# grossmanlev/FL-distributed-delay

Measured on AMD Instinct MI355X. Metric: simulated worker-steps/sec (node) @1024 workers, delay 50; aggregation HBM GB/s, higher is better.
Workload: dtype f32

## Files before the change

### fl-distributed-delay_amd/csrc/gemm_core.h

```cpp
#pragma once
#include <type_traits>

#include "common.h"

namespace flsim {

constexpr int GK = 16;

__device__ __forceinline__ int kc_swz(int row) { return (4 - ((row >> 2) & 3)) & 3; }

template <int ROWS>
struct KCTile {
    static constexpr int FLOATS = ROWS * GK;
    __device__ static inline int chunk_off(int row, int chunk) {
        return row * GK + 4 * (chunk ^ kc_swz(row));
    }
};
template <int ROWS>
struct KMTile {
    static constexpr int STRIDE = ROWS + 4;
    static constexpr int DUMMY = GK * STRIDE;
    static constexpr int FLOATS = GK * STRIDE + 4;
};

__device__ __forceinline__ f32x4 mfma16(float a, float b, f32x4 c) {
    return __builtin_amdgcn_mfma_f32_16x16x4f32(a, b, c, 0, 0, 0);
}

template <bool KC, int ROWS>
__device__ __forceinline__ f32x4 read_frag(const float* lds, int r0, int lane) {
    if constexpr (KC) {
        const int row = r0 + (lane & 15);
        return *reinterpret_cast<const f32x4*>(lds + KCTile<ROWS>::chunk_off(row, lane >> 4));
    } else {
        constexpr int S = KMTile<ROWS>::STRIDE;
        const int col = r0 + (lane & 15);
        const int k0 = 4 * (lane >> 4);
        f32x4 v;
        v.x = lds[(k0 + 0) * S + col];
        v.y = lds[(k0 + 1) * S + col];
        v.z = lds[(k0 + 2) * S + col];
        v.w = lds[(k0 + 3) * S + col];
        return v;
    }
}

template <bool KC, int ROWS>
__device__ __forceinline__ void store_unit(float* lds, int a, int b, f32x4 v) {
    if constexpr (KC) {
        *reinterpret_cast<f32x4*>(lds + KCTile<ROWS>::chunk_off(a, b)) = v;
    } else {
        *reinterpret_cast<f32x4*>(lds + a * KMTile<ROWS>::STRIDE + 4 * b) = v;
    }
}

template <int ROWS>
__device__ __forceinline__ void store_km_or_spare(float* lds, bool valid, int a, int b, f32x4 v) {
    const int off = valid ? a * KMTile<ROWS>::STRIDE + 4 * b : KMTile<ROWS>::DUMMY;
    *reinterpret_cast<f32x4*>(lds + off) = v;
}

template <bool KC, int ROWS>
constexpr int tile_floats() {
    if constexpr (KC) return KCTile<ROWS>::FLOATS;
    else return KMTile<ROWS>::FLOATS;
}


template <class E, class = void>
struct IsStaged : std::false_type {};
template <class E>
struct IsStaged<E, std::void_t<decltype(E::STAGED)>> : std::bool_constant<E::STAGED> {};

template <class E, class = void>
struct IsPartial : std::false_type {};
template <class E>
struct IsPartial<E, std::void_t<decltype(E::PARTIAL)>> : std::bool_constant<E::PARTIAL> {};

template <class EPI>
__device__ __forceinline__ void staged_store(const EPI& epi, const float* tile, int ld, int m0,
                                             int bm, int n0, int bn, int tid, int nt) {
    if constexpr (IsPartial<EPI>::value)
        epi.store_rows(tile, ld, m0, bm, n0, bn, tid, nt);
    else
        epi.store_rows(tile, ld, m0, bm, tid, nt);
}

template <class E, class = void>
struct HasPre : std::false_type {};
template <class E>
struct HasPre<E, std::void_t<decltype(E::PRE)>> : std::bool_constant<E::PRE> {};

#ifndef FLSIM_SINGLE_BUF
#define FLSIM_SINGLE_BUF 2
#endif

template <int FM, int FN, int WAVES_M, int WAVES_N, class AL, class BL, class EPI>
__global__ void __launch_bounds__(64 * WAVES_M * WAVES_N)
gemm_kernel(AL al, BL bl, EPI epi, int ksteps_total, int ksteps_per_split, int tiles_m,
            int tiles_n) {
    constexpr int BM = 16 * FM * WAVES_M;
    constexpr int BN = 16 * FN * WAVES_N;
    static_assert(AL::ROWS == BM, "A loader rows != BM");
    static_assert(BL::ROWS == BN, "B loader rows != BN");
    constexpr int A_FL = tile_floats<AL::KC, BM>();
    constexpr int B_FL = tile_floats<BL::KC, BN>();
    constexpr bool STAGED = IsStaged<EPI>::value;
    constexpr int STAGE_LD = BN + 4;
    constexpr bool SB = WAVES_M * WAVES_N <= FLSIM_SINGLE_BUF && !STAGED;
    constexpr int BASE_FL = (SB ? 1 : 2) * (A_FL + B_FL);
    constexpr int STAGE_BUDGET = BASE_FL > 8192 ? BASE_FL : 8192;
    constexpr int WROWS = 16 * FM;
    constexpr int WM_FIT = STAGE_BUDGET / (WROWS * STAGE_LD);
    constexpr int WM_PASS = WM_FIT < 1 ? 1 : (WM_FIT > WAVES_M ? WAVES_M : WM_FIT);
    constexpr int LDS_FL = STAGED && WM_PASS * WROWS * STAGE_LD > BASE_FL
                               ? WM_PASS * WROWS * STAGE_LD : BASE_FL;
    __shared__ __attribute__((aligned(16))) float lds[LDS_FL];

    const int tid = threadIdx.x;
    const int lane = tid & 63;
    const int wave = tid >> 6;
    const int wm = wave / WAVES_N;
    const int wn = wave % WAVES_N;
    const int gx = tiles_m, gy = tiles_n;
    const int nb = gridDim.x;
    const int b = blockIdx.x;
    const int q = nb / 8, r = nb % 8, xcd = b % 8;
    const int L = (xcd < r ? xcd * (q + 1) : r * (q + 1) + (xcd - r) * q) + b / 8;
    const int tn = L % gy;
    const int tm = (L / gy) % gx;
    const int tz = L / (gx * gy);
    const int m0 = tm * BM;
    const int n0 = tn * BN;
    const int ks0 = tz * ksteps_per_split;
    int ks1 = ks0 + ksteps_per_split;
    if (ks1 > ksteps_total) ks1 = ksteps_total;

    al.setup(m0, tid);
    bl.setup(n0, tid);

    f32x4 acc[FM][FN];
#pragma unroll
    for (int i = 0; i < FM; ++i)
#pragma unroll
        for (int j = 0; j < FN; ++j) acc[i][j] = f32x4{0.f, 0.f, 0.f, 0.f};

    float asum = 0.f;
    f32x4 ra[AL::UNITS];
    f32x4 rb[BL::UNITS];
    constexpr int BUF = A_FL + B_FL;

    if (ks0 < ks1) {
        al.load(ks0, ra);
        bl.load(ks0, rb);
        if constexpr (!SB) {
            al.store(lds, ra);
            bl.store(lds + A_FL, rb);
            if (ks0 + 1 < ks1) {
                al.load(ks0 + 1, ra);
                bl.load(ks0 + 1, rb);
            }
        }
    }
    __syncthreads();
    if constexpr (WAVES_M * WAVES_N == 8) {
        if (wave >= 4) __builtin_amdgcn_s_setprio(1);
    }
    int cur = 0;
    for (int ks = ks0; ks < ks1; ++ks) {
        if constexpr (SB) {
            al.store(lds, ra);
            bl.store(lds + A_FL, rb);
            if (ks + 1 < ks1) {
                al.load(ks + 1, ra);
                bl.load(ks + 1, rb);
            }
            __syncthreads();
        } else if (ks + 1 < ks1) {
            al.store(lds + (cur ^ 1) * BUF, ra);
            bl.store(lds + (cur ^ 1) * BUF + A_FL, rb);
            if (ks + 2 < ks1) {
                al.load(ks + 2, ra);
                bl.load(ks + 2, rb);
            }
        }
        const float* A = lds + (SB ? 0 : cur * BUF);
        const float* B = A + A_FL;
        if constexpr (EPI::ASUM) {
            static_assert(!AL::KC, "ASUM needs a k-major A tile");
            if (tn == 0 && tid < BM) {
#pragma unroll
                for (int k = 0; k < GK; ++k) asum += A[k * KMTile<BM>::STRIDE + tid];
            }
        }
        f32x4 af[FM], bf[FN];
#pragma unroll
        for (int i = 0; i < FM; ++i) af[i] = read_frag<AL::KC, BM>(A, wm * 16 * FM + 16 * i, lane);
#pragma unroll
        for (int j = 0; j < FN; ++j) bf[j] = read_frag<BL::KC, BN>(B, wn * 16 * FN + 16 * j, lane);
#pragma unroll
        for (int kk = 0; kk < 4; ++kk)
#pragma unroll
            for (int i = 0; i < FM; ++i)
#pragma unroll
                for (int j = 0; j < FN; ++j) acc[i][j] = mfma16(af[i][kk], bf[j][kk], acc[i][j]);
        __syncthreads();
        cur ^= 1;
    }

    if constexpr (EPI::ASUM) {
        if (tn == 0 && tid < BM) epi.asum(m0 + tid, tz, asum);
    }
    if constexpr (STAGED) {
        static_assert(BN == EPI::NCOL || (IsPartial<EPI>::value && EPI::NCOL % BN == 0),
                      "staged epilogue needs the full row in one block");
        constexpr int PASSES = (WAVES_M + WM_PASS - 1) / WM_PASS;
#pragma unroll 1
        for (int pass = 0; pass < PASSES; ++pass) {
            __syncthreads();
            if (wm / WM_PASS == pass) {
#pragma unroll
                for (int i = 0; i < FM; ++i)
#pragma unroll
                    for (int j = 0; j < FN; ++j) {
                        const int ml = (wm - pass * WM_PASS) * WROWS + 16 * i + 4 * (lane >> 4);
                        const int nl = wn * 16 * FN + 16 * j + (lane & 15);
#pragma unroll
                        for (int r = 0; r < 4; ++r)
                            lds[(ml + r) * STAGE_LD + nl] = epi.value(nl, acc[i][j][r]);
                    }
            }
            __syncthreads();
            const int wm_hi = (pass + 1) * WM_PASS < WAVES_M ? (pass + 1) * WM_PASS : WAVES_M;
            staged_store(epi, lds, STAGE_LD, m0 + pass * WM_PASS * WROWS,
                         (wm_hi - pass * WM_PASS) * WROWS, n0, BN, tid, 64 * WAVES_M * WAVES_N);
        }
    } else if constexpr (HasPre<EPI>::value) {
#pragma unroll
        for (int i = 0; i < FM; ++i) {
            const int m = m0 + wm * 16 * FM + 16 * i + 4 * (lane >> 4);
            const int nb = n0 + wn * 16 * FN + (lane & 15);
            f32x4 pre[FN];
#pragma unroll
            for (int j = 0; j < FN; ++j) pre[j] = epi.pre4(m, nb + 16 * j, tz);
#pragma unroll
            for (int j = 0; j < FN; ++j) epi.apply4p(m, nb + 16 * j, tz, acc[i][j], pre[j]);
        }
    } else {
#pragma unroll
        for (int i = 0; i < FM; ++i)
#pragma unroll
            for (int j = 0; j < FN; ++j) {
                const int m = m0 + wm * 16 * FM + 16 * i + 4 * (lane >> 4);
                const int n = n0 + wn * 16 * FN + 16 * j + (lane & 15);
                epi.apply4(m, n, tz, acc[i][j]);
            }
    }
}

}
```

### fl-distributed-delay_amd/csrc/loaders.h

```cpp
#pragma once
#include "gemm_core.h"
#include "pn1.h"
#include "split.h"

namespace flsim {

__device__ __forceinline__ f32x4 ldg4(const float* p) { return *reinterpret_cast<const f32x4*>(p); }
__device__ __forceinline__ f32x4 zero4() { return f32x4{0.f, 0.f, 0.f, 0.f}; }
__device__ __forceinline__ void st_nt4(float* p, f32x4 v) {
    __builtin_nontemporal_store(v, reinterpret_cast<f32x4*>(p));
}

__device__ __forceinline__ f32x4 ldg4_or0(const float* p, const float* , bool ok) {
    return ok ? ldg4(p) : zero4();
}

#ifndef FLSIM_BUFLOAD
#define FLSIM_BUFLOAD 1
#endif
constexpr unsigned BUF_OOB = 0xfffffff0u;
__device__ __forceinline__ __amdgpu_buffer_rsrc_t raw_rsrc(const void* base, unsigned long bytes) {
    const unsigned n = bytes < (unsigned long)BUF_OOB ? (unsigned)bytes : BUF_OOB;
    return __builtin_amdgcn_make_buffer_rsrc(const_cast<void*>(base), (short)0, (int)n, 0x00020000);
}
// ... 319 lines not shown
struct Im2colKM {
    using Unit = typename SRC::Unit;
    static constexpr int ROWS = TR;
    static constexpr bool KC = false;
    static constexpr int OH = VO > 0 ? VO : IH + 2 * PAD - 2;
    static constexpr int OW = VO > 0 ? VO : IW + 2 * PAD - 2;
    static constexpr int C4 = ROWS / 4;
    static constexpr int TPR = NT / GK;
    static_assert(NT % GK == 0, "");
    static constexpr int UNITS = (C4 + TPR - 1) / TPR;
    static_assert(FLSIM_BUFLOAD || !SRC::SPLIT, "split operands use buffer loads");
    static constexpr int PIX = SRC::SM ? GK : CI;
    static constexpr int SLICE = SRC::SM ? IH * IW * GK : GK;
    static_assert(!SRC::SM || CI % GK == 0, "slice-major maps have whole 16-channel slices");
    const float* X;
    const float* XL = nullptr;
    int M;
    int krow;
    int coff[UNITS];
    short kh[UNITS], kw[UNITS];
    short c4[UNITS];
    SRC buf;
    __device__ void setup(int c0, int tid) {
        krow = km_row<TPR>(tid);
        if constexpr (FLSIM_BUFLOAD)
            buf.init(X, XL, (unsigned long)((M + OH * OW - 1) / (OH * OW)) * IH * IW * CI * 4);
#pragma unroll
        for (int j = 0; j < UNITS; ++j) {
            const int c = tid % TPR + TPR * j;
            c4[j] = (short)c;
            const int kk = c0 + 4 * c;
            const int khkw = kk / CI;
            const int ci = kk - khkw * CI;
            const bool real = c < C4 && khkw < 9;
            kh[j] = (short)(real ? khkw / 3 : -64);
            kw[j] = (short)(khkw % 3);
            coff[j] = real ? ((khkw / 3 - PAD) * IW + (khkw % 3 - PAD)) * PIX + (ci / GK) * SLICE +
                                 ci % GK
                           : 0;
        }
    }
    __device__ void load(int ks, Unit (&r)[UNITS]) const {
        const int p = ks * GK + krow;
        const unsigned img0 = (unsigned)(ks * GK) / (unsigned)(OH * OW);
        unsigned rem = (unsigned)(ks * GK) - img0 * (OH * OW) + krow, img = img0;
        if constexpr (OH * OW >= GK) {
            if (rem >= (unsigned)(OH * OW)) { rem -= OH * OW; ++img; }
        } else {
            const unsigned q = SmallDiv<OH * OW, OH * OW + GK>::div(rem);
            img += q;
            rem -= q * (OH * OW);
        }
        const int oh = (int)SmallDiv<OW, OH * OW + GK>::div(rem);
        const int ow = (int)rem - oh * OW;
        const bool pok = p < M;
        if constexpr (FLSIM_BUFLOAD) {
            const unsigned xb = img * (unsigned)(IH * IW * CI * 4) + (unsigned)(oh * IW + ow) * (PIX * 4u);
#pragma unroll
            for (int j = 0; j < UNITS; ++j) {
                const int ih = oh + kh[j] - PAD, iw = ow + kw[j] - PAD;
                const bool ok = pok && (unsigned)ih < (unsigned)IH && (unsigned)iw < (unsigned)IW;
                r[j] = buf.ld_or0(xb + (unsigned)coff[j] * 4u, ok);
            }
        } else {
            static_assert(!SRC::SM, "slice-major maps use buffer loads");
            const long xo = ((long)img * IH * IW + oh * IW + ow) * CI;
#pragma unroll
            for (int j = 0; j < UNITS; ++j) {
                const int ih = oh + kh[j] - PAD, iw = ow + kw[j] - PAD;
                const bool ok = pok && (unsigned)ih < (unsigned)IH && (unsigned)iw < (unsigned)IW;
                r[j] = ldg4_or0(X + xo + coff[j], X, ok);
            }
        }
    }
    __device__ void store(float* lds, const f32x4 (&r)[UNITS]) const {
#pragma unroll
        for (int j = 0; j < UNITS; ++j)
            store_km_or_spare<ROWS>(lds, C4 % TPR == 0 || c4[j] < C4, krow, c4[j], r[j]);
    }
    template <class F>
    __device__ void each_unit(const Unit (&r)[UNITS], F&& f) const {
#pragma unroll
        for (int j = 0; j < UNITS; ++j) f(krow, c4[j], r[j], C4 % TPR == 0 || c4[j] < C4);
    }
};

struct EpiBias {
    static constexpr bool ASUM = false;
    float* Y;
    const float* bias;
    int M, N;
    __device__ void apply4(int m, int n, int z, f32x4 v) const {
        if (n >= N) return;
        const float b = bias[n];
#pragma unroll
        for (int r = 0; r < 4; ++r)
            if (m + r < M) Y[(long)(m + r) * N + n] = v[r] + b;
    }
};

struct EpiBiasRelu {
    static constexpr bool ASUM = false;
    float* Y;
    const float* bias;
    int M, N;
    __device__ void apply4(int m, int n, int z, f32x4 v) const {
        if (n >= N) return;
        const float b = bias[n];
#pragma unroll
        for (int r = 0; r < 4; ++r)
            if (m + r < M) Y[(long)(m + r) * N + n] = fmaxf(v[r] + b, 0.f);
    }
};

template <int NC>
struct EpiBiasReluRows {
    static constexpr bool ASUM = false;
    static constexpr bool STAGED = true;
    static constexpr int NCOL = NC;
    static_assert(NC % 4 == 0, "float4 rows");
    float* Y;
    const float* bias;
    int M;
    __device__ float value(int n, float v) const { return fmaxf(v + bias[n], 0.f); }
    __device__ void store_rows(const float* tile, int ld, int m0, int bm, int tid, int nt) const {
        const int rows = M - m0 < bm ? M - m0 : bm;
        constexpr int N4 = NC / 4;
        f32x4* dst = reinterpret_cast<f32x4*>(Y + (long)m0 * NC);
        for (int q = tid; q < rows * N4; q += nt) {
            const int r = q / N4, c = q - r * N4;
            st_nt4(reinterpret_cast<float*>(dst + q), *reinterpret_cast<const f32x4*>(tile + r * ld + 4 * c));
        }
    }
};

template <int PH, int PW, int C, bool NCHW_OUT>
struct EpiPoolDrop {
    static constexpr bool ASUM = false;
    float* d;
    uint8_t* idx;
    const float* bias;
    const WorkerRec* workers;
    uint64_t seed;
    uint32_t site, thr;
    float scale;
    int dropout;
    int M;
    __device__ void apply4(int m, int n, int z, f32x4 v) const {
        if (n >= C || m >= M) return;
        const float b = bias[n];
        float mv = fmaxf(v[0] + b, 0.f);
        int mi = 0;
#pragma unroll
        for (int r = 1; r < 4; ++r) {
            const float x = fmaxf(v[r] + b, 0.f);
            if (x > mv) { mv = x; mi = r; }
        }
        const int q = m >> 2;
        const int pw = q % PW;
        const int ph = (q / PW) % PH;
        const int s = q / (PW * PH);
        const int w = s / SAMPLES_PER_WORKER;
        const int nl = s - w * SAMPLES_PER_WORKER;
        float out = mv;
        if (dropout) {
            const WorkerRec wr = workers[w];
// ... 121 lines not shown
    __device__ void store_rows(const float* tile, int ld, int m0, int bm, int tid, int nt) const {
        const int rows = M - m0 < bm ? M - m0 : bm;
        constexpr int N4 = NC / 4;
        const f32x4* a4 = reinterpret_cast<const f32x4*>(act + (long)m0 * NC);
        const uint32_t* i4 = reinterpret_cast<const uint32_t*>(idx + (long)m0 * NC);
        const int total = rows * N4;
        int q0 = tid;
        if constexpr (BATCH > 0) {
            f32x4 av[BATCH];
            uint32_t iv[BATCH];
#pragma unroll
            for (int it = 0; it < BATCH; ++it) {
                const int q = tid + it * nt;
                if (q < total) {
                    av[it] = a4[q];
                    iv[it] = i4[q];
                }
            }
#pragma unroll
            for (int it = 0; it < BATCH; ++it) {
                const int q = tid + it * nt;
                if (q < total) unit(tile, ld, m0, q, av[it], iv[it]);
            }
            q0 = tid + BATCH * nt;
        }
        for (int q = q0; q < total; q += nt) unit(tile, ld, m0, q, a4[q], i4[q]);
    }
    __device__ void unit(const float* tile, int ld, int m0, int q, f32x4 a, uint32_t id) const {
        constexpr int N4 = NC / 4;
        {
            const int r = q / N4, c = q - r * N4;
            const f32x4 t = *reinterpret_cast<const f32x4*>(tile + r * ld + 4 * c);
            f32x4 g;
            g.x = a.x > 0.f ? t.x * scale : 0.f;
            g.y = a.y > 0.f ? t.y * scale : 0.f;
            g.z = a.z > 0.f ? t.z * scale : 0.f;
            g.w = a.w > 0.f ? t.w * scale : 0.f;
            const unsigned mm = (unsigned)(m0 + r);
            const unsigned img = mm / (PH * PW);
            const unsigned rem = mm - img * (PH * PW);
            const unsigned ph = rem / PW, pw = rem - ph * PW;
            float* base = dZ + (((long)img * (2 * PH) + 2 * ph) * (2 * PW) + 2 * pw) * NC + 4 * c;
#pragma unroll
            for (int pos = 0; pos < 4; ++pos) {
                f32x4 o;
                o.x = (id & 0xffu) == (uint32_t)pos ? g.x : 0.f;
                o.y = ((id >> 8) & 0xffu) == (uint32_t)pos ? g.y : 0.f;
                o.z = ((id >> 16) & 0xffu) == (uint32_t)pos ? g.z : 0.f;
                o.w = (id >> 24) == (uint32_t)pos ? g.w : 0.f;
                st_nt4(base + ((pos >> 1) * (2 * PW) + (pos & 1)) * (long)NC, o);
            }
        }
    }
};

struct EpiSlabAcc {
    static constexpr bool ASUM = true;
    static constexpr bool ASUM_MFMA = true;
    float* S;
    int M, N;
    long zstride;
    float* Bsl;
    int zinit = 0x7fffffff;
    __device__ void asum(int m, int z, float v) const {
        if (!Bsl || m >= M) return;
        if (z < zinit) Bsl[(long)z * M + m] += v;
        else Bsl[(long)z * M + m] = v;
    }
    __device__ void apply4(int m, int n, int z, f32x4 v) const {
        if (n >= N) return;
        float* base = S + z * zstride;
        if (z < zinit) {
#pragma unroll
            for (int r = 0; r < 4; ++r)
                if (m + r < M) base[(long)(m + r) * N + n] += v[r];
        } else {
#pragma unroll
            for (int r = 0; r < 4; ++r)
                if (m + r < M) base[(long)(m + r) * N + n] = v[r];
        }
    }
};

struct EpiSlabStore {
    static constexpr bool ASUM = false;
    float* S;
    int M, N;
    long zstride;
    __device__ void apply4(int m, int n, int z, f32x4 v) const {
        if (n >= N) return;
        float* base = S + z * zstride;
#pragma unroll
        for (int r = 0; r < 4; ++r)
            if (m + r < M) base[(long)(m + r) * N + n] = v[r];
    }
};

struct EpiSlabStoreFresh : EpiSlabStore {
    static constexpr bool X6_FRESH = true;
};

}
```

### fl-distributed-delay_amd/csrc/net_kernels.h

```cpp
#pragma once
#include "epi_xs.h"
#include "gemm_direct.h"
#include "gemm_dx6.h"
#include "gemm_x6.h"
#include "loaders.h"
#include "pn1.h"
#include "probe.h"

namespace flsim {

static __global__ void __launch_bounds__(256)
k_fill_batch(const uint8_t* __restrict__ pool, const int32_t* __restrict__ labels,
             const int32_t* __restrict__ list_a, int len_a, const int32_t* __restrict__ list_b,
             int len_b, const WorkerRec* __restrict__ workers, int n_workers_total, uint64_t seed,
             const float* __restrict__ lut, float* __restrict__ x0, int32_t* __restrict__ y) {
    const int s = blockIdx.x;
    const int w = s / SAMPLES_PER_WORKER;
    const int j = s - w * SAMPLES_PER_WORKER;
    const WorkerRec wr = workers[w];
    const uint32_t bsz = wr.pad ? wr.pad : (uint32_t)SAMPLES_PER_WORKER;
    const uint32_t q = (wr.i >> 20) * SAMPLES_PER_WORKER + (uint32_t)j;
    float* out = x0 + (long)s * 4096;
    if (q >= bsz) {
        if (threadIdx.x == 0) y[s] = -1;
// ... 711 lines not shown
        int dev = 0;
        if (hipGetDevice(&dev) != hipSuccess ||
            hipDeviceGetAttribute(&cus, hipDeviceAttributeMultiprocessorCount, dev) != hipSuccess)
            cus = -1;
    }
    int per = 0;
    if (cus <= 0 || hipOccupancyMaxActiveBlocksPerMultiprocessor(&per, f, nt, 0) != hipSuccess)
        return 0;
    return per * cus;
}

template <int IH, int IW, int CI, int PAD, int FM, int FN, int WM, int WN, class EPI, int OHX = 0,
          bool X6 = false>
static int conv_like(const float* X, int S, const float* Wpk, int N, int KP, const EPI& epi,
                     hipStream_t st, int kid, int kreal) {
    constexpr int NT = 64 * WM * WN;
    constexpr int BM = 16 * FM * WM, BN = 16 * FN * WN;
    using AL = Im2colKC<IH, IW, CI, PAD, BM, NT, false, OHX>;
    using BL = RowsKC<BN, NT>;
    AL al;
    al.X = X;
    al.M = S * AL::OH * AL::OW;
    BL bl;
    bl.P = Wpk;
    bl.ld = KP;
    bl.NR = N;
    return launch_gemm<FM, FN, WM, WN, X6>(al, bl, epi, al.M, N, KP / GK, 1, st, kid,
                                           2.0 * al.M * N * kreal);
}

template <int IH, int IW, int CI, int PAD, int FM, int FN, int WM, int WN, int OHX = 0, class EPI>
static int conv_x6(const float* X, int S, const float* Wpk, int N, int KP, const EPI& epi,
                   hipStream_t st, int kid, int kreal) {
    return conv_like<IH, IW, CI, PAD, FM, FN, WM, WN, EPI, OHX, true>(X, S, Wpk, N, KP, epi, st,
                                                                      kid, kreal);
}

template <int IH, int IW, int CI, int PAD, int FM, int FMS, int FN, int WM, int WN, class EPI>
static int conv_like_sz(const float* X, int S, const float* Wpk, int N, int KP, const EPI& epi,
                        hipStream_t st, int kid, int kreal) {
    if (S <= small_chunk_samples())
        return conv_like<IH, IW, CI, PAD, FMS, FN, WM, WN>(X, S, Wpk, N, KP, epi, st, kid, kreal);
    return conv_like<IH, IW, CI, PAD, FM, FN, WM, WN>(X, S, Wpk, N, KP, epi, st, kid, kreal);
}

template <int IH, int IW, int CI, int PAD, int FM, int FN, int WM, int WN, int VO = 0,
          bool DZC = false, bool X6 = false, class SRC = BufSrc, class SRCB = SRC>
static int conv_wgrad(const float* dz, const float* X, int S, int CO, int KP, float* slab,
                      float* bslab, int Z, hipStream_t st, int kid, int kreal,
                      int zinit = 0x7fffffff, int* zused = nullptr, const float* dzl = nullptr,
                      const float* Xl = nullptr) {
    constexpr int NT = 64 * WM * WN;
    constexpr int BM = 16 * FM * WM, BN = 16 * FN * WN;
    constexpr int OFULL = IH + 2 * PAD - 2;
    static_assert(IH == IW && VO <= OFULL, "square maps only");
    static_assert(X6 || (!SRC::SPLIT && !SRCB::SPLIT), "split operands run on the split-bf16 GEMM");
    using AL = RowsKM<BM, NT, (VO > 0 && !DZC ? OFULL : 0), (DZC ? 0 : VO), SRC>;
    using BL = Im2colKM<IH, IW, CI, PAD, BN, NT, VO, SRCB>;
    const int M = S * BL::OH * BL::OW;
    AL al;
    al.P = dz;
    al.PL = dzl;
    al.ld = CO;
    al.NK = M;
    al.NC = CO;
    BL bl;
    bl.X = X;
    bl.XL = Xl;
    bl.M = M;
    EpiSlabAcc epi{slab, CO, KP, (long)CO * KP, bslab, zinit};
    const int tiles = ceil_div(CO, BM) * ceil_div(KP, BN);
    const void* kfn;
    if constexpr (X6)
        kfn = (const void*)gemm_x6_kernel<FM, FN, WM, WN, AL, BL, EpiSlabAcc>;
    else
        kfn = (const void*)gemm_kernel<FM, FN, WM, WN, AL, BL, EpiSlabAcc>;
    static const int cap = resident_blocks(kfn, NT);
    const int zu = wsplit(ceil_div(M, GK), Z, tiles, cap);
    if (zused) *zused = zu;
    return launch_gemm<FM, FN, WM, WN, X6>(al, bl, epi, CO, KP, ceil_div(M, GK), zu, st, kid,
                                           2.0 * M * CO * kreal);
}

template <int IH, int IW, int CI, int PAD, int FM, int FN, int WM, int WN, int FMS, int FNS,
          int WMS, int WNS, int VO = 0, bool DZC = false, bool X6 = false, class SRC = BufSrc,
          class SRCB = SRC>
static int conv_wgrad_sz(const float* dz, const float* X, int S, int CO, int KP, float* slab,
                         float* bslab, int Z, hipStream_t st, int kid, int kreal, int zinit,
                         int* zused, const float* dzl = nullptr, const float* Xl = nullptr) {
    if (S <= small_chunk_samples())
        return conv_wgrad<IH, IW, CI, PAD, FMS, FNS, WMS, WNS, VO, DZC, X6, SRC, SRCB>(
            dz, X, S, CO, KP, slab, bslab, Z, st, kid, kreal, zinit, zused, dzl, Xl);
    return conv_wgrad<IH, IW, CI, PAD, FM, FN, WM, WN, VO, DZC, X6, SRC, SRCB>(
        dz, X, S, CO, KP, slab, bslab, Z, st, kid, kreal, zinit, zused, dzl, Xl);
}

template <int IH, int IW, int CI, int PAD, int FM, int FN, int WAVES, int KB, int DEPTH, int NPL,
          bool WIN, int OHX, class ASRC = XsSrc, class EPI>
static int conv_dx6(XsT X, int S, XsT W, int N, int KP, const EPI& epi, hipStream_t st, int kid,
                    int kreal) {
    static_assert(ASRC::SPLIT, "split input");
    using AD = Im2colDirect<IH, IW, CI, PAD, FM, WIN, OHX, ASRC>;
    using BL = RowsKCStageXs<16 * FN, 64 * WAVES, NPL>;
    constexpr int BM = 16 * FM * WAVES, BN = 16 * FN;
    FLSIM_REQUIRE((KP / GK) % KB == 0, "direct GEMM: %d k-steps not a multiple of %d", KP / GK, KB);
    AD ad;
    ad.X = X.hm;
    ad.XL = X.l;
    ad.M = S * AD::ROWS_PER_IMG;
    BL bl;
    bl.P = W.hm;
    bl.PL = W.l;
    bl.ld = KP;
    bl.NR = N;
    const int tm = ceil_div(ad.M, BM), tn = ceil_div(N, BN);
    const ProbeSlot ps = probe_begin();
    hipExtLaunchKernelGGL((gemm_dx6_kernel<FM, FN, WAVES, KB, DEPTH, AD, BL, EPI>),
                          dim3(tm * tn), dim3(64 * WAVES), 0, st, ps.start, ps.stop, 0, ad, bl,
                          epi, KP / GK, tm, tn);
    FLSIM_LAUNCH_CHECK();
    return probe_end(ps, kid, 2.0 * ad.M * N * kreal);
}

template <int IH, int IW, int CI, int PAD, int FM, int FN, int WM, int WN, bool WIN, int OHX,
          class EPI>
static int conv_xs(XsT X, int S, XsT W, int N, int KP, const EPI& epi, hipStream_t st, int kid,
                   int kreal) {
    constexpr int NT = 64 * WM * WN;
    constexpr int BM = 16 * FM * WM, BN = 16 * FN * WN;
    using AL = Im2colKC<IH, IW, CI, PAD, BM, NT, WIN, OHX, XsSrc>;
    using BL = RowsKC<BN, NT, XsSrc>;
    AL al;
    al.X = X.hm;
    al.XL = X.l;
    al.M = S * AL::ROWS_PER_IMG;
    BL bl;
    bl.P = W.hm;
    bl.PL = W.l;
    bl.ld = KP;
    bl.NR = N;
    return launch_gemm<FM, FN, WM, WN, true>(al, bl, epi, al.M, N, KP / GK, 1, st, kid,
                                             2.0 * al.M * N * kreal);
}

template <int IH, int IW, int CI, int CO, int PAD, int FM, int FN, int WM, int WN, bool NCHW_OUT,
          bool X6 = false>
static int conv_pool_fwd(const float* X, int S, const float* Wpk, int KP, float* d, uint8_t* idx,
                         const float* bias, const WorkerRec* workers, uint64_t seed, uint32_t site,
                         uint32_t thr, float scale, int dropout, hipStream_t st, int kid,
                         int kreal) {
    constexpr int NT = 64 * WM * WN;
    constexpr int BM = 16 * FM * WM, BN = 16 * FN * WN;
    using AL = Im2colKC<IH, IW, CI, PAD, BM, NT, true>;
    using BL = RowsKC<BN, NT>;
    AL al;
    al.X = X;
    al.M = S * AL::ROWS_PER_IMG;
    BL bl;
    bl.P = Wpk;
    bl.ld = KP;
    bl.NR = CO;
    EpiPoolDrop<AL::PH, AL::PW, CO, NCHW_OUT> epi{d, idx, bias, workers, seed, site, thr,
                                                  scale, dropout, al.M};
    return launch_gemm<FM, FN, WM, WN, X6>(al, bl, epi, al.M, CO, KP / GK, 1, st, kid,
                                           2.0 * al.M * CO * kreal);
}
// ... 46 lines not shown
```

### fl-distributed-delay_amd/csrc/pn1_net.hip

```cpp
#include <stdarg.h>
#include <stdio.h>
#include <string.h>

#include <mutex>
#include <unordered_map>

#include "net_kernels.h"
#include "slabstep.h"

namespace flsim {

static thread_local char g_err[512];
void set_error(const char* fmt, ...) {
    va_list ap;
    va_start(ap, fmt);
    vsnprintf(g_err, sizeof(g_err), fmt, ap);
    va_end(ap);
}
const char* last_error() { return g_err; }

struct ConvGeo {
    int CI, CIP, CO, H;
    int KP;
    int ZW;
// ... 330 lines not shown
    auto it = g_pipes.find(gradstate);
    if (it == g_pipes.end() || !it->second.pending) return 0;
    Pipe& p = it->second;
    FLSIM_CHECK_HIP(hipEventRecord(p.bwd_tail, p.bs));
    FLSIM_CHECK_HIP(hipStreamWaitEvent(st, p.bwd_tail, 0));
    p.pending = false;
    return 0;
}

static void pipe_release(const void* gradstate) {
    std::lock_guard<std::mutex> lk(g_pipe_mu);
    auto it = g_pipes.find(gradstate);
    if (it == g_pipes.end()) return;
    Pipe& p = it->second;
    (void)hipStreamSynchronize(p.bs);
    for (auto& kv : p.ws_free) (void)hipEventDestroy(kv.second);
    (void)hipEventDestroy(p.fwd_done);
    (void)hipEventDestroy(p.bwd_tail);
    (void)hipStreamDestroy(p.bs);
    g_pipes.erase(it);
}

static StepPlan plan_in_use(const GradState& g, const void* gradstate) {
    const EpochRows* er = epoch_rows(gradstate);
    if (!er) return g.plan;
    SegSpec specs[STEP_MAX_SEG];
    const int n = pn1_segments(g, reinterpret_cast<const float*>(gradstate), specs);
    int zin[STEP_MAX_SEG];
    for (int i = 0; i < n; ++i) {
        zin[i] = specs[i].Z;
        if (specs[i].group >= 0) {
            const int z = er->z[specs[i].group];
            zin[i] = z < specs[i].Z ? z : specs[i].Z;
            specs[i].Z = zin[i] > 0 ? zin[i] : 1;
        }
    }
    StepPlan p;
    plan_step(specs, n, &p);
    for (int i = 0; i < p.nseg; ++i)
        for (int j = 0; j < n; ++j)
            if (specs[j].slab_off == p.seg[i].slab_off) p.seg[i].zlim = zin[j];
    return p;
}

struct SideStream {
    hipStream_t s = nullptr;
    hipEvent_t to_side = nullptr, to_main = nullptr;
    std::mutex* mu = nullptr;
};
static SideStream* side_stream() {
    static std::mutex mu;
    static std::unordered_map<int, SideStream> per_dev;
    int dev = 0;
    if (hipGetDevice(&dev) != hipSuccess) return nullptr;
    std::lock_guard<std::mutex> lk(mu);
    SideStream& ss = per_dev[dev];
    if (!ss.s) {
        if (hipStreamCreateWithFlags(&ss.s, hipStreamNonBlocking) != hipSuccess ||
            hipEventCreateWithFlags(&ss.to_side, hipEventDisableTiming) != hipSuccess ||
            hipEventCreateWithFlags(&ss.to_main, hipEventDisableTiming) != hipSuccess) {
            ss = SideStream{};
            return nullptr;
        }
        ss.mu = new std::mutex();
    }
    return &ss;
}
static bool concurrent_backward(int S) {
    static int smax = -1;
    if (smax < 0) {
        const char* e = lab_env("FLSIM_CONCURRENT_BWD");
        smax = e ? atoi(e) : 2048;
    }
    return S <= smax;
}

#ifndef FLSIM_DG_FMS
#define FLSIM_DG_FMS 2
#endif
constexpr int DG_FMS = FLSIM_DG_FMS;

#ifndef FLSIM_WGRAD_X6
#define FLSIM_WGRAD_X6 0
#endif

static int debug_stop() {
    const char* e = getenv("FLSIM_DEBUG_BWD_STOP");
    return e ? atoi(e) : 0;
}

static int backward(const GradState& g, const WS& w, const float* theta, int S, int dropout,
                    hipStream_t st, EpochRows* er) {
    constexpr int ALL = 0x7fffffff;
    auto zi = [&](int grp) { return er ? er->z[grp] : ALL; };
    int zu[8] = {0, 0, 0, 0, 0, 0, 0, 0};
    const float s25 = dropout ? SCALE_P25 : 1.f;
    const float s50 = dropout ? SCALE_P50 : 1.f;
    SideStream* ss = concurrent_backward(S) ? side_stream() : nullptr;
    std::unique_lock<std::mutex> ss_lock;
    if (ss) ss_lock = std::unique_lock<std::mutex>(*ss->mu);
    hipStream_t sw = ss ? ss->s : st;
    auto fork = [&]() -> int {
        if (!ss) return 0;
        FLSIM_CHECK_HIP(hipEventRecord(ss->to_side, st));
        FLSIM_CHECK_HIP(hipStreamWaitEvent(ss->s, ss->to_side, 0));
        return 0;
    };
    auto join = [&]() -> int {
        if (!ss) return 0;
        FLSIM_CHECK_HIP(hipEventRecord(ss->to_main, ss->s));
        FLSIM_CHECK_HIP(hipStreamWaitEvent(st, ss->to_main, 0));
        return 0;
    };
    auto finish = [&]() -> int {
        RC(join());
        if (er)
            for (int i = 0; i < 8; ++i)
                if (zu[i] > er->z[i]) er->z[i] = zu[i];
        return 0;
    };
    RC(head_wgrad<256>(w.dlog, w.e2, g.l3w, g.l3b, S, ZH, st));
    RC(fork());
    RC((linear_wgrad<4, 4, 2, 2>(w.dh2, w.e1, g.l2w, g.l2b, S, 256, 512, ZL2W, sw, K_L2W, zi(7),
                                 &zu[7])));
    RC((linear_dgrad<2, 2, 2, 2>(w.dh2, theta + P_OFF[14], w.dh1, w.e1, s50, S, 256, 512, st,
                                 K_L2D)));
    RC(fork());
    RC((linear_wgrad<4, 4, 2, 2, true>(w.dh1, w.d3, g.l1w, g.l1b, S, 512, 9408, ZL1W, sw, K_L1W,
                                       zi(6), &zu[6])));
    if (S <= 2048)
        RC((linear_dgrad<2, 4, 2, 2>(w.dh1, theta + P_OFF[12], w.gy, w.d3, s25, S, 512, 9408, st,
                                     K_L1D)));
    else
        RC((linear_dgrad<4, 4, 2, 2>(w.dh1, theta + P_OFF[12], w.gy, w.d3, s25, S, 512, 9408, st,
                                     K_L1D)));
    RC((pool_scatter<14, 14, 192, true>(w.gy, w.i3, w.a6, S, st)));
    float* const dz6 = w.a6;
    float* const dz5 = w.gx;
    float* const dz4 = w.a4;
    RC(fork());
#if FLSIM_WGRAD_X6
    RC((conv_wgrad_sz<13, 13, 192, 2, 6, 3, 2, 2, 3, 3, 2, 2, 14, true, true, BufSrc, XsSrc>(
        dz6, w.a5, S, 192, 1728, g.sw[5], g.sb[5], GEO[5].ZW, sw, K_WG6, 1728, zi(5), &zu[5],
        nullptr, w.a5l)));
#else
    RC((conv_wgrad<13, 13, 192, 2, 6, 3, 2, 4, 14, true, false, BufSrc, BufSrc>(
        dz6, w.a5f, S, 192, 1728, g.sw[5], g.sb[5], GEO[5].ZW, sw, K_WG6, 1728, zi(5), &zu[5])));
#endif
    RC((conv_direct_sz<14, 14, 192, 0, 2, DG_FMS, 6, 8, 6, 2, false, 13>(dz6, S, g.wd[5], 192, 1728,
        EpiMaskXs<192, false>{dz5, nullptr, w.a5, S * 13 * 13}, st, K_DG6, 1728)));
    if (debug_stop() == 6) return finish();
    RC(fork());
#if FLSIM_WGRAD_X6
    RC((conv_wgrad_sz<11, 11, 96, 2, 6, 3, 2, 2, 3, 3, 2, 2, 0, false, true, BufSrc, XsSrc>(
        dz5, w.d2, S, 192, 864, g.sw[4], g.sb[4], GEO[4].ZW, sw, K_WG5, 864, zi(4), &zu[4],
        nullptr, w.d2l)));
#else
    RC((conv_wgrad<11, 11, 96, 2, 6, 3, 2, 2, 0, false, false, BufSrc, BufSrc>(
        dz5, w.d2f, S, 192, 864, g.sw[4], g.sb[4], GEO[4].ZW, sw, K_WG5, 864, zi(4), &zu[4])));
#endif
    RC((conv_direct_sz<13, 13, 192, 0, 2, DG_FMS, 6, 8, 3, 2, false, 0>(dz5, S, g.wd[4], 96, 1728,
        EpiDropScatterXs<11, 11, 96, false>{dz4, nullptr, w.d2, w.i2, s25, S * 11 * 11}, st,
        K_DG5, 1728)));
    if (debug_stop() == 5) return finish();
    RC(join());
    RC(fork());
#if FLSIM_WGRAD_X6
    RC((conv_wgrad<20, 20, 96, 2, 3, 3, 2, 2, 0, false, true, BufSrc, XsSrcSM>(
        dz4, w.a3, S, 96, 864, g.sw[3], g.sb[3], GEO[3].ZW, sw, K_WG4, 864, zi(3), &zu[3],
        nullptr, w.a3l)));
#else
    RC((conv_wgrad<20, 20, 96, 2, 3, 3, 2, 2, 0, false, false, BufSrc, BufSrcSM>(
        dz4, w.a3f, S, 96, 864, g.sw[3], g.sb[3], GEO[3].ZW, sw, K_WG4, 864, zi(3), &zu[3])));
#endif
    RC((conv_direct_sz<22, 22, 96, 0, 2, DG_FMS, 6, 8, 3, 2, false, 0>(dz4, S, g.wd[3], 96, 864,
        EpiMaskXs<96, false, true, 400>{w.gx, nullptr, w.a3, S * 20 * 20}, st, K_DG4, 864)));
    if (debug_stop() == 4) return finish();
    float* dz3 = w.gx;
    RC(fork());
#if FLSIM_WGRAD_X6
    RC((conv_wgrad_sz<18, 18, 48, 2, 3, 3, 2, 2, 3, 3, 2, 2, 0, false, true, BufSrc, XsSrcSM>(
        dz3, w.d1, S, 96, 432, g.sw[2], g.sb[2], GEO[2].ZW, sw, K_WG3, 432, zi(2), &zu[2],
        nullptr, w.d1l)));
#else
    RC((conv_wgrad<18, 18, 48, 2, 3, 3, 2, 1, 0, false, false, BufSrc, BufSrcSM>(
        dz3, w.d1f, S, 96, 432, g.sw[2], g.sb[2], GEO[2].ZW, sw, K_WG3, 432, zi(2), &zu[2])));
#endif
#ifndef FLSIM_DG3_FM
#define FLSIM_DG3_FM 2
#endif
    RC((conv_like_sz<20, 20, 96, 0, FLSIM_DG3_FM, 2, 3, 4, 1>(dz3, S, g.wd[2], 48, 864,
        EpiDropScatterXs<18, 18, 48, false, true>{w.a2, nullptr, w.d1, w.i1, s25, S * 18 * 18}, st,
        K_DG3, 864)));
    if (debug_stop() == 3) return finish();
    float* dz2 = w.a2;
    RC(join());
    RC(fork());
#if FLSIM_WGRAD_X6
    RC((conv_wgrad_sz<34, 34, 48, 2, 3, 3, 1, 3, 3, 3, 1, 3, 0, false, true, BufSrc, XsSrcSM>(
        dz2, w.a1, S, 48, 432, g.sw[1], g.sb[1], GEO[1].ZW, sw, K_WG2, 432, zi(1), &zu[1],
        nullptr, w.a1l)));
#else
    RC((conv_wgrad<34, 34, 48, 2, 3, 3, 1, 1, 0, false, false, BufSrc, BufSrcSM>(
        dz2, w.a1f, S, 48, 432, g.sw[1], g.sb[1], GEO[1].ZW, sw, K_WG2, 432, zi(1), &zu[1])));
#endif
    RC((conv_direct_sz<36, 36, 48, 0, 2, 1, 3, 8, 3, 2, false, 0>(dz2, S, g.wd[1], 48, 432,
        EpiMaskXs<48, false, true, 1156>{w.gx, nullptr, w.a1, S * 34 * 34}, st, K_DG2, 432)));
    float* dz1 = w.gx;
    RC((conv_wgrad<32, 32, 4, 2, 1, 3, 3, 1>(dz1, w.x0, S, 48, 48, g.sw[0], g.sb[0], GEO[0].ZW,
                                            st, K_WG1, 27, zi(0), &zu[0])));
    return finish();
}

}

using namespace flsim;

extern "C" {

const char* flsim_last_error(void) { return last_error(); }

long flsim_pn1_param_count(void) { return P_TOTAL; }

long flsim_pn1_gradstate_bytes(void) { return gs_layout(nullptr).total_floats * 4; }

long flsim_pn1_workspace_bytes(int max_samples) { return ws_layout(nullptr, max_samples).bytes; }

int flsim_pn1_workspace_offset(int which, int samples, long* offset_bytes) {
    char* const fake = reinterpret_cast<char*>(4096);
    WS w = ws_layout(fake, samples);
    const void* p[] = {w.x0, w.a1, w.a2, w.d1, w.a3, w.a4, w.d2, w.a5, w.a6, w.d3,
                       w.e1, w.e2, w.dh1, w.dh2, w.gx, w.gy, w.loss_s, w.dlog, w.y,
                       w.i1, w.i2, w.i3,
                       w.a1l, w.d1l, w.a3l, w.d2l, w.a5l, w.a6l, w.a4l, w.a2l, w.gxl,
                       w.a1f, w.d1f, w.a3f, w.d2f, w.a5f};
    FLSIM_REQUIRE(which >= 0 && which < (int)(sizeof(p) / sizeof(p[0])), "bad workspace id %d", which);
    *offset_bytes = (long)((const char*)p[which] - fake);
    return 0;
}

int flsim_pn1_workspace_split_part(int which) {
    switch (which) {
        case 1: return 22;
        case 3: return 23;
        case 4: return 24;
        case 6: return 25;
        case 7: return 26;
        default: return -1;
    }
}

int flsim_pn1_workspace_slice_major(int which) {
    return which == 1 || which == 3 || which == 4;
}

int flsim_pn1_begin_epoch(void* gradstate, const float* theta, hipStream_t stream) {
    FLSIM_REQUIRE(gradstate && theta, "null pointer");
    RC(pipe_join(gradstate, stream));
    GradState g = gs_layout((float*)gradstate);
    RC(pack_weights(g, theta, stream));
    FLSIM_CHECK_HIP(hipMemsetAsync(g.l3w, 0, (g.l3b + ZH * 10 - g.l3w) * 4, stream));
    FLSIM_CHECK_HIP(hipMemsetAsync((float*)gradstate + g.cnt_off, 0,
                                   step_counter_floats(g.plan) * 4, stream));
    std::lock_guard<std::mutex> lk(g_rows_mu);
    g_rows[gradstate] = EpochRows{{0, 0, 0, 0, 0, 0, 0, 0}};
    return 0;
}

void flsim_pn1_release(void* gradstate) {
    pipe_release(gradstate);
    std::lock_guard<std::mutex> lk(g_rows_mu);
    g_rows.erase(gradstate);
}

static int run_chunk(void* gradstate, const WS& w, const float* theta, const WorkerRec* workers,
                     int n_chunk_workers, uint64_t seed, int dropout, int backward_pass,
                     float* worker_loss, hipStream_t stream,
                     float gscale = 1.f / SAMPLES_PER_WORKER) {
    const int S = n_chunk_workers * SAMPLES_PER_WORKER;
    GradState g = gs_layout((float*)gradstate);
    RC(forward(g, w, theta, S, workers, seed, dropout, stream));
    RC(head_and_loss<256>(w.e2, theta + P_OFF[16], theta + P_OFF[17], w.y, w.loss_s, w.dlog, w.dh2,
                          S, backward_pass, dropout ? SCALE_P50 : 1.f, gscale, worker_loss,
                          stream, workers));
// ... 319 lines not shown
```

Before: 1111.

## Add dense weight-gradient GEMM that reads dZ per tap instead of im2col

Adds a weight-gradient path where each n-tile is one 3x3 filter tap. The A loader reads the padded dZ map shifted by that tap, and the B loader reads the layer input pixels directly. This avoids building an im2col-style expanded operand. The bias gradient is now computed on the last n-tile, with an extra ring-sum pass that adds the dZ values in the padding border which the shifted reads miss. The path is enabled by default for layers 3 to 6. The cost is extra loads and LDS syncs for the border sum, and different tiling per layer.

Measured after the change: 1176 (median of 6 runs). 5.8% higher.

```diff
diff --git a/fl-distributed-delay_amd/csrc/gemm_core.h b/fl-distributed-delay_amd/csrc/gemm_core.h
--- a/fl-distributed-delay_amd/csrc/gemm_core.h
+++ b/fl-distributed-delay_amd/csrc/gemm_core.h
@@ -90,6 +90,16 @@
 struct HasPre : std::false_type {};
 template <class E>
 struct HasPre<E, std::void_t<decltype(E::PRE)>> : std::bool_constant<E::PRE> {};
+
+template <class L, class = void>
+struct WantsN0 : std::false_type {};
+template <class L>
+struct WantsN0<L, std::void_t<decltype(L::WANTS_N0)>> : std::bool_constant<L::WANTS_N0> {};
+
+template <class E, class = void>
+struct HasBiasRing : std::false_type {};
+template <class E>
+struct HasBiasRing<E, std::void_t<decltype(E::BIAS_RING)>> : std::bool_constant<E::BIAS_RING> {};
 
 #ifndef FLSIM_SINGLE_BUF
 #define FLSIM_SINGLE_BUF 2
@@ -136,7 +146,9 @@
     int ks1 = ks0 + ksteps_per_split;
     if (ks1 > ksteps_total) ks1 = ksteps_total;
 
-    al.setup(m0, tid);
+    const int asum_tn = HasBiasRing<EPI>::value ? gy - 1 : 0;
+    if constexpr (WantsN0<AL>::value) al.setup(m0, tid, n0);
+    else al.setup(m0, tid);
     bl.setup(n0, tid);
 
     f32x4 acc[FM][FN];
@@ -146,6 +158,10 @@
         for (int j = 0; j < FN; ++j) acc[i][j] = f32x4{0.f, 0.f, 0.f, 0.f};
 
     float asum = 0.f;
+    if constexpr (HasBiasRing<EPI>::value) {
+        static_assert(AL::RING_FLOATS <= LDS_FL, "the ring's partial sums fit the pipeline's LDS");
+        if (tn == asum_tn) asum = al.bias_ring(ks0, ks1, m0, tid, lds);
+    }
     f32x4 ra[AL::UNITS];
     f32x4 rb[BL::UNITS];
     constexpr int BUF = A_FL + B_FL;
@@ -188,7 +204,7 @@
         const float* B = A + A_FL;
         if constexpr (EPI::ASUM) {
             static_assert(!AL::KC, "ASUM needs a k-major A tile");
-            if (tn == 0 && tid < BM) {
+            if (tn == asum_tn && tid < BM) {
 #pragma unroll
                 for (int k = 0; k < GK; ++k) asum += A[k * KMTile<BM>::STRIDE + tid];
             }
@@ -209,7 +225,7 @@
     }
 
     if constexpr (EPI::ASUM) {
-        if (tn == 0 && tid < BM) epi.asum(m0 + tid, tz, asum);
+        if (tn == asum_tn && tid < BM) epi.asum(m0 + tid, tz, asum);
     }
     if constexpr (STAGED) {
         static_assert(BN == EPI::NCOL || (IsPartial<EPI>::value && EPI::NCOL % BN == 0),
diff --git a/fl-distributed-delay_amd/csrc/loaders.h b/fl-distributed-delay_amd/csrc/loaders.h
--- a/fl-distributed-delay_amd/csrc/loaders.h
+++ b/fl-distributed-delay_amd/csrc/loaders.h
@@ -425,6 +425,175 @@
     __device__ void each_unit(const Unit (&r)[UNITS], F&& f) const {
 #pragma unroll
         for (int j = 0; j < UNITS; ++j) f(krow, c4[j], r[j], C4 % TPR == 0 || c4[j] < C4);
+    }
+};
+
+template <int PIXELS>
+__device__ __forceinline__ void km_pixel(int ks, int krow, unsigned& img, unsigned& rem) {
+    static_assert(PIXELS >= GK, "one image carry at most per k-step");
+    img = (unsigned)(ks * GK) / (unsigned)PIXELS;
+    rem = (unsigned)(ks * GK) - img * PIXELS + krow;
+    if (rem >= (unsigned)PIXELS) { rem -= PIXELS; ++img; }
+}
+
+template <int IH, int IW, int CI, int DH, int TR, int NT, class SRC = BufSrc>
+struct TapRowsKM {
+    using Unit = typename SRC::Unit;
+    static_assert(!SRC::SM && !SRC::SPLIT, "pixel-major fp32 dZ");
+    static_assert(FLSIM_BUFLOAD, "buffer loads only");
+    static_assert(DH == IH + 2 || DH == IH + 1, "padding 2: full map, or compact by one row/column");
+    static constexpr int ROWS = TR;
+    static constexpr bool KC = false;
+    static constexpr bool WANTS_N0 = true;
+    static constexpr bool EDGE = DH < IH + 2;
+    static constexpr int C4 = ROWS / 4;
+    static constexpr int TPR = NT / GK;
+    static_assert(NT % GK == 0, "");
+    static constexpr int UNITS = (C4 + TPR - 1) / TPR;
+    static constexpr int GROUPS = NT / C4;
+    static constexpr int RING_FLOATS = GROUPS * ROWS;
+    static constexpr int RING_AHEAD = 4;
+    static_assert(GROUPS >= 1, "");
+    const float* P;
+    long ld;
+    int M;
+    int NC;
+    int krow;
+    int dh, dw;
+    int c_off[UNITS];
+    short c4[UNITS];
+    SRC buf;
+    __device__ unsigned long bytes() const {
+        return (unsigned long)(M / (IH * IW)) * (DH * DH) * ld * 4;
+    }
+    __device__ void setup(int c0, int tid, int n0) {
+        krow = km_row<TPR>(tid);
+        buf.init(P, bytes());
+        const int tap = n0 / CI;
+        dh = 2 - tap / 3;
+        dw = 2 - tap % 3;
+#pragma unroll
+        for (int j = 0; j < UNITS; ++j) {
+            const int c = tid % TPR + TPR * j;
+            c4[j] = (short)c;
+            const int col = c0 + 4 * c;
+            c_off[j] = (c < C4 && col < NC) ? col : -1;
+        }
+    }
+    __device__ void load(int ks, Unit (&r)[UNITS]) const {
+        unsigned img, rem;
+        km_pixel<IH * IW>(ks, krow, img, rem);
+        const unsigned ih = SmallDiv<IW, IH * IW + GK>::div(rem);
+        const unsigned oh = ih + dh, ow = rem - ih * IW + dw;
+        bool rok = ks * GK + krow < M;
+        if constexpr (EDGE) rok = rok && oh < (unsigned)DH && ow < (unsigned)DH;
+        const unsigned rb = (img * (unsigned)(DH * DH) + oh * DH + ow) * ((unsigned)ld * 4u);
+#pragma unroll
+        for (int j = 0; j < UNITS; ++j)
+            r[j] = buf.ld_or0(rb + (unsigned)c_off[j] * 4u, rok && c_off[j] >= 0);
+    }
+    __device__ void store(float* lds, const f32x4 (&r)[UNITS]) const {
+#pragma unroll
+        for (int j = 0; j < UNITS; ++j)
+            store_km_or_spare<ROWS>(lds, C4 % TPR == 0 || c4[j] < C4, krow, c4[j], r[j]);
+    }
+    __device__ float bias_ring(int ks0, int ks1, int c0, int tid, float* lds) const {
+        constexpr int P = IH * IW, RN = DH * DH - P;
+        constexpr int BOTTOM = (DH - IH) * DH;
+        constexpr int RW = DH - IW;
+        const int q0 = ks0 * GK;
+        int q1 = ks1 * GK < M ? ks1 * GK : M;
+        if (q1 < q0) q1 = q0;
+        const int i0 = (q0 + P - 1) / P, i1 = (q1 + P - 1) / P;
+        const int total = (i1 - i0) * RN;
+        const int g = tid / C4, c = tid - g * C4;
+        const int col = c0 + 4 * c;
+        const unsigned rstride = (unsigned)ld * 4u;
+        auto off = [&](int idx) -> unsigned {
+            const unsigned img = (unsigned)idx / (unsigned)RN;
+            const unsigned r = (unsigned)idx - img * RN;
+            unsigned pix = IH * DH + r;
+            if (r >= (unsigned)BOTTOM) {
+                const unsigned r2 = r - BOTTOM, oh = r2 / RW;
+                pix = oh * DH + IW + (r2 - oh * RW);
+            }
+            return ((i0 + img) * (unsigned)(DH * DH) + pix) * rstride + (unsigned)col * 4u;
+        };
+        f32x4 s = zero4();
+        if (g < GROUPS && col < NC) {
+            int i = g;
+            for (; i + (RING_AHEAD - 1) * GROUPS < total; i += RING_AHEAD * GROUPS) {
+                f32x4 v[RING_AHEAD];
+#pragma unroll
+                for (int j = 0; j < RING_AHEAD; ++j) v[j] = buf.ld(off(i + j * GROUPS));
+#pragma unroll
+                for (int j = 0; j < RING_AHEAD; ++j) s += v[j];
+            }
+            for (; i < total; i += GROUPS) s += buf.ld(off(i));
+        }
+        if (g < GROUPS) *reinterpret_cast<f32x4*>(lds + g * ROWS + 4 * c) = s;
+        __syncthreads();
+        float t = 0.f;
+        if (tid < ROWS) {
+            t = lds[tid];
+#pragma unroll
+            for (int i = 1; i < GROUPS; ++i) t += lds[i * ROWS + tid];
+        }
+        __syncthreads();
+        return t;
+    }
+};
+
+template <int IH, int IW, int CI, int TR, int NT, class SRC = BufSrc>
+struct PixRowsKM {
+    using Unit = typename SRC::Unit;
+    static_assert(!SRC::SPLIT, "fp32 layer input");
+    static_assert(FLSIM_BUFLOAD, "buffer loads only");
+    static_assert(!SRC::SM || CI % GK == 0, "slice-major maps have whole 16-channel slices");
+    static constexpr int ROWS = TR;
+    static constexpr bool KC = false;
+    static constexpr int C4 = ROWS / 4;
+    static constexpr int TPR = NT / GK;
+    static_assert(NT % GK == 0, "");
+    static constexpr int UNITS = (C4 + TPR - 1) / TPR;
+    static constexpr int PIX = SRC::SM ? GK : CI;
+    static constexpr int SLICE = SRC::SM ? IH * IW * GK : GK;
+    const float* X;
+    int M;
+    int krow;
+    int coff[UNITS];
+    short c4[UNITS];
+    SRC buf;
+    __device__ void setup(int n0, int tid) {
+        krow = km_row<TPR>(tid);
+        buf.init(X, (unsigned long)M * CI * 4);
+        const int ci0 = n0 % CI;
+#pragma unroll
+        for (int j = 0; j < UNITS; ++j) {
+            const int c = tid % TPR + TPR * j;
+            c4[j] = (short)c;
+            const int ci = ci0 + 4 * c;
+            coff[j] = (c < C4 && ci < CI) ? (ci / GK) * SLICE + ci % GK : -1;
+        }
+    }
+    __device__ void load(int ks, Unit (&r)[UNITS]) const {
+        const int q = ks * GK + krow;
+        unsigned xb;
+        if constexpr (SRC::SM) {
+            unsigned img, rem;
+            km_pixel<IH * IW>(ks, krow, img, rem);
+            xb = img * (unsigned)(IH * IW * CI * 4) + rem * (PIX * 4u);
+        } else {
+            xb = (unsigned)q * (CI * 4u);
+        }
+#pragma unroll
+        for (int j = 0; j < UNITS; ++j)
+            r[j] = buf.ld_or0(xb + (unsigned)coff[j] * 4u, q < M && coff[j] >= 0);
+    }
+    __device__ void store(float* lds, const f32x4 (&r)[UNITS]) const {
+#pragma unroll
+        for (int j = 0; j < UNITS; ++j)
+            store_km_or_spare<ROWS>(lds, C4 % TPR == 0 || c4[j] < C4, krow, c4[j], r[j]);
     }
 };
 
@@ -712,6 +881,10 @@
     }
 };
 
+struct EpiSlabAccRing : EpiSlabAcc {
+    static constexpr bool BIAS_RING = true;
+};
+
 struct EpiSlabStore {
     static constexpr bool ASUM = false;
     float* S;
diff --git a/fl-distributed-delay_amd/csrc/net_kernels.h b/fl-distributed-delay_amd/csrc/net_kernels.h
--- a/fl-distributed-delay_amd/csrc/net_kernels.h
+++ b/fl-distributed-delay_amd/csrc/net_kernels.h
@@ -817,6 +817,41 @@
                                            2.0 * M * CO * kreal);
 }
 
+template <int IH, int IW, int CI, int FM, int FN, int WM, int WN, int DH, class SRCB = BufSrc>
+static int conv_wgrad_dense(const float* dz, const float* X, int S, int CO, int KP, float* slab,
+                            float* bslab, int Z, hipStream_t st, int kid, int kreal,
+                            int zinit = 0x7fffffff, int* zused = nullptr) {
+    constexpr int NT = 64 * WM * WN;
+    constexpr int BM = 16 * FM * WM, BN = 16 * FN * WN;
+    static_assert(IH == IW, "square maps only");
+    static_assert(BN == CI, "an n-tile is exactly one filter tap");
+    using AL = TapRowsKM<IH, IW, CI, DH, BM, NT>;
+    using BL = PixRowsKM<IH, IW, CI, BN, NT, SRCB>;
+    FLSIM_REQUIRE(KP == 9 * CI, "dense weight gradient: %d columns, not 9 taps of %d", KP, CI);
+    const int M = S * IH * IW;
+    AL al;
+    al.P = dz;
+    al.ld = CO;
+    al.M = M;
+    al.NC = CO;
+    BL bl;
+    bl.X = X;
+    bl.M = M;
+    EpiSlabAccRing epi{{slab, CO, KP, (long)CO * KP, bslab, zinit}};
+    const int tm = ceil_div(CO, BM), tn = KP / BN;
+    static const int cap =
+        resident_blocks((const void*)gemm_kernel<FM, FN, WM, WN, AL, BL, EpiSlabAccRing>, NT);
+    const int ksteps = ceil_div(M, GK);
+    const int zu = wsplit(ksteps, Z, tm * tn, cap);
+    if (zused) *zused = zu;
+    const int per = (ksteps + zu - 1) / zu;
+    const ProbeSlot ps = probe_begin();
+    hipExtLaunchKernelGGL((gemm_kernel<FM, FN, WM, WN, AL, BL, EpiSlabAccRing>), dim3(tm * tn * zu),
+                          dim3(NT), 0, st, ps.start, ps.stop, 0, al, bl, epi, ksteps, per, tm, tn);
+    FLSIM_LAUNCH_CHECK();
+    return probe_end(ps, kid, 2.0 * M * CO * kreal);
+}
+
 template <int IH, int IW, int CI, int PAD, int FM, int FN, int WM, int WN, int FMS, int FNS,
           int WMS, int WNS, int VO = 0, bool DZC = false, bool X6 = false, class SRC = BufSrc,
           class SRCB = SRC>
diff --git a/fl-distributed-delay_amd/csrc/pn1_net.hip b/fl-distributed-delay_amd/csrc/pn1_net.hip
--- a/fl-distributed-delay_amd/csrc/pn1_net.hip
+++ b/fl-distributed-delay_amd/csrc/pn1_net.hip
@@ -436,6 +436,22 @@
 
 #ifndef FLSIM_WGRAD_X6
 #define FLSIM_WGRAD_X6 0
+#endif
+
+#ifndef FLSIM_WGD2
+#define FLSIM_WGD2 0
+#endif
+#ifndef FLSIM_WGD3
+#define FLSIM_WGD3 1
+#endif
+#ifndef FLSIM_WGD4
+#define FLSIM_WGD4 1
+#endif
+#ifndef FLSIM_WGD5
+#define FLSIM_WGD5 1
+#endif
+#ifndef FLSIM_WGD6
+#define FLSIM_WGD6 1
 #endif
 
 static int debug_stop() {
@@ -497,6 +513,9 @@
     RC((conv_wgrad_sz<13, 13, 192, 2, 6, 3, 2, 2, 3, 3, 2, 2, 14, true, true, BufSrc, XsSrc>(
         dz6, w.a5, S, 192, 1728, g.sw[5], g.sb[5], GEO[5].ZW, sw, K_WG6, 1728, zi(5), &zu[5],
         nullptr, w.a5l)));
+#elif FLSIM_WGD6
+    RC((conv_wgrad_dense<13, 13, 192, 6, 3, 2, 4, 14>(
+        dz6, w.a5f, S, 192, 1728, g.sw[5], g.sb[5], GEO[5].ZW, sw, K_WG6, 1728, zi(5), &zu[5])));
 #else
     RC((conv_wgrad<13, 13, 192, 2, 6, 3, 2, 4, 14, true, false, BufSrc, BufSrc>(
         dz6, w.a5f, S, 192, 1728, g.sw[5], g.sb[5], GEO[5].ZW, sw, K_WG6, 1728, zi(5), &zu[5])));
@@ -509,6 +528,9 @@
     RC((conv_wgrad_sz<11, 11, 96, 2, 6, 3, 2, 2, 3, 3, 2, 2, 0, false, true, BufSrc, XsSrc>(
         dz5, w.d2, S, 192, 864, g.sw[4], g.sb[4], GEO[4].ZW, sw, K_WG5, 864, zi(4), &zu[4],
         nullptr, w.d2l)));
+#elif FLSIM_WGD5
+    RC((conv_wgrad_dense<11, 11, 96, 6, 3, 2, 2, 13>(
+        dz5, w.d2f, S, 192, 864, g.sw[4], g.sb[4], GEO[4].ZW, sw, K_WG5, 864, zi(4), &zu[4])));
 #else
     RC((conv_wgrad<11, 11, 96, 2, 6, 3, 2, 2, 0, false, false, BufSrc, BufSrc>(
         dz5, w.d2f, S, 192, 864, g.sw[4], g.sb[4], GEO[4].ZW, sw, K_WG5, 864, zi(4), &zu[4])));
@@ -523,6 +545,9 @@
     RC((conv_wgrad<20, 20, 96, 2, 3, 3, 2, 2, 0, false, true, BufSrc, XsSrcSM>(
         dz4, w.a3, S, 96, 864, g.sw[3], g.sb[3], GEO[3].ZW, sw, K_WG4, 864, zi(3), &zu[3],
         nullptr, w.a3l)));
+#elif FLSIM_WGD4
+    RC((conv_wgrad_dense<20, 20, 96, 3, 3, 2, 2, 22, BufSrcSM>(
+        dz4, w.a3f, S, 96, 864, g.sw[3], g.sb[3], GEO[3].ZW, sw, K_WG4, 864, zi(3), &zu[3])));
 #else
     RC((conv_wgrad<20, 20, 96, 2, 3, 3, 2, 2, 0, false, false, BufSrc, BufSrcSM>(
         dz4, w.a3f, S, 96, 864, g.sw[3], g.sb[3], GEO[3].ZW, sw, K_WG4, 864, zi(3), &zu[3])));
@@ -536,6 +561,9 @@
     RC((conv_wgrad_sz<18, 18, 48, 2, 3, 3, 2, 2, 3, 3, 2, 2, 0, false, true, BufSrc, XsSrcSM>(
         dz3, w.d1, S, 96, 432, g.sw[2], g.sb[2], GEO[2].ZW, sw, K_WG3, 432, zi(2), &zu[2],
         nullptr, w.d1l)));
+#elif FLSIM_WGD3
+    RC((conv_wgrad_dense<18, 18, 48, 3, 3, 2, 1, 20, BufSrcSM>(
+        dz3, w.d1f, S, 96, 432, g.sw[2], g.sb[2], GEO[2].ZW, sw, K_WG3, 432, zi(2), &zu[2])));
 #else
     RC((conv_wgrad<18, 18, 48, 2, 3, 3, 2, 1, 0, false, false, BufSrc, BufSrcSM>(
         dz3, w.d1f, S, 96, 432, g.sw[2], g.sb[2], GEO[2].ZW, sw, K_WG3, 432, zi(2), &zu[2])));
@@ -554,6 +582,9 @@
     RC((conv_wgrad_sz<34, 34, 48, 2, 3, 3, 1, 3, 3, 3, 1, 3, 0, false, true, BufSrc, XsSrcSM>(
         dz2, w.a1, S, 48, 432, g.sw[1], g.sb[1], GEO[1].ZW, sw, K_WG2, 432, zi(1), &zu[1],
         nullptr, w.a1l)));
+#elif FLSIM_WGD2
+    RC((conv_wgrad_dense<34, 34, 48, 3, 3, 1, 1, 36, BufSrcSM>(
+        dz2, w.a1f, S, 48, 432, g.sw[1], g.sb[1], GEO[1].ZW, sw, K_WG2, 432, zi(1), &zu[1])));
 #else
     RC((conv_wgrad<34, 34, 48, 2, 3, 3, 1, 1, 0, false, false, BufSrc, BufSrcSM>(
         dz2, w.a1f, S, 48, 432, g.sw[1], g.sb[1], GEO[1].ZW, sw, K_WG2, 432, zi(1), &zu[1])));
```
